# JiahaoPlus/EvoWorld

Measured on AMD Instinct MI355X. Metric: panoramic frames/sec per clip (576x1024x25f, 25 denoise steps), higher is better.
Workload: dtype f16

## Files before the change

### evoworld_amd/_model.py

```python
import json
import math
import os
from collections import OrderedDict
from types import SimpleNamespace

import torch

from . import ops
from .ops import A_CONV3X3, A_CONVT3


class Spec(OrderedDict):

    def add(self, name, shape, kind):
        self[name] = (tuple(shape), kind)

    def conv(self, p, o, i, k):
        self.add(p + ".weight", (o, i) + k, i * math.prod(k))
        self.add(p + ".bias", (o,), i * math.prod(k))

    def lin(self, p, o, i, bias=True):
        self.add(p + ".weight", (o, i), i)
        if bias:
            self.add(p + ".bias", (o,), i)

    def norm(self, p, c):
        self.add(p + ".weight", (c,), "gamma")
        self.add(p + ".bias", (c,), "beta")


class Weights:

    def __init__(self, sd, device):
        self.sd, self.device = sd, device

    def f32(self, k):
        return self.sd[k].to(device=self.device, dtype=torch.float32)

    @staticmethod
    def h(t):
        return t.to(torch.float16).contiguous()

    def pair(self, p):
        return self.h(self.f32(p + ".weight")), self.h(self.f32(p + ".bias"))

    def conv(self, p, cpad=None):
        return ops.pack_conv_weight(self.f32(p + ".weight"), cpad), self.h(self.f32(p + ".bias"))


class PackedModel:
    DEFAULTS = {}
    WEIGHT_FILES = ()
    MISSING = "state dict is missing"
    _spec = _random = None
    PRETRAINED_KW = ()

    def __init__(self, cfg, dtype):
        self._cfg = cfg
        self.config = SimpleNamespace(**cfg)
        self.dtype = dtype
        self.device, self.w = None, None

    @classmethod
    def _config_from_json(cls, raw):
        return {k: raw[k] for k in cls.DEFAULTS if k in raw}

    @classmethod
    def read_config(cls, root):
        cj = os.path.join(root, "config.json")
        if not os.path.exists(cj):
# ... 30 lines not shown
        self.device = torch.device(device)
        if self.device.type != "cuda":
            raise RuntimeError(f"evoworld_amd.{type(self).__name__} needs a GPU device (no CPU path)")
        self._pack(sd)
        return self

    def _require_loaded(self):
        if self.w is None:
            raise RuntimeError("weights not loaded")

    def to(self, *a, **k):
        return self

    def eval(self):
        return self

    def requires_grad_(self, _flag=False):
        return self

    def _conv3x3(self, x, w, b, N, H, W_, Ho, Wo, stride=1, upsample=0, res_out=False, x2=None, c2=None, **kw):
        c1 = x.shape[-1]
        lda2 = x2.shape[-1] if x2 is not None else 0
        M = N * Ho * Wo
        out = self._res(M, w.shape[0], x.device, head="r1" not in kw) if res_out else torch.empty(M, w.shape[0], dtype=torch.float16, device=x.device)
        return ops.gemm(x, w, out, M=M, N=w.shape[0], c1=c1, lda=c1, a2=x2, c2=lda2 if c2 is None else c2, lda2=lda2, bias=b,
                        mode=A_CONV3X3, conv=(N, H, W_, Ho, Wo, stride, upsample), **kw)

    def _convt(self, x, w, b, B, T, P, res_out=False, **kw):
        C = x.shape[-1]
        M = B * T * P
        out = self._res(M, w.shape[0], x.device) if res_out else torch.empty(M, w.shape[0], dtype=torch.float16, device=x.device)
        return ops.gemm(x, w, out, M=M, N=w.shape[0], c1=C, lda=C, bias=b, mode=A_CONVT3, tconv=(B, T, P), **kw)
```

### evoworld_amd/csrc/gemm3_f16.hip

```cpp
#include "gemm_gen23.h"

namespace {

#define EW3_LDS(ptr) (*(const f16x8*)(ptr))

#ifndef EW3_BN
#define EW3_BN 320
#endif
#if EW3_BN == 320
#define EW3_NAME(x) x
#define EW3_KERNEL_STR "gemm3_kernel"
#else
#define EW3_NAME(x) x##_b256
#define EW3_KERNEL_STR "gemm3b_kernel"
#define gemm3_kernel gemm3b_kernel
#endif
constexpr int BM = 256, BN = EW3_BN, BK = 64, NW = 8, WAVES_N = 2;
constexpr int WM = 64, WN = BN / WAVES_N, FM = 4, FN = WN / 16;
static_assert(BN % 64 == 0 && FN % 2 == 0 && (FM * FN) % 8 == 0, "tile geometry");
constexpr int A_BYTES = BM * 128, STAGE = (BM + BN) * 128;
constexpr int GA = BM / 8 / NW, GB = BN / 8 / NW, NP = GA + GB;
constexpr int NSTEP = 2 * FN;
constexpr int ITEMS_BYTES = 8192;
constexpr int PD = 2;
constexpr int BAR_STEP = NSTEP - 1 - PD;


__device__ __forceinline__ void tile_coords(int id, int tiles_m, int tiles_n, int band, int& tm, int& tn) {
    if (band <= 0 || tiles_n <= band) { tm = id / tiles_n; tn = id - tm * tiles_n; return; }
    const int nb = (tiles_n + band - 1) / band;
    const int per_band = band * tiles_m;
    const int k = min(id / per_band, nb - 1);
    const int r = id - k * per_band;
    const int w = k == nb - 1 ? tiles_n - k * band : band;
    tm = r / w;
    tn = k * band + (r - tm * w);
}

template <int MODE, int EPI>
__global__ __launch_bounds__(64 * NW, 2) void gemm3_kernel(const GemmP p, const SkP sk) {
    extern __shared__ __attribute__((aligned(16))) char smem[];
    constexpr bool DIRECT = (EPI & 8) == 0 && (MODE == EW_A_DENSE || (EPI & 16));
#ifndef EW_G3_RESLDS
#define EW_G3_RESLDS 1
#endif
    constexpr bool RB_INIT = DIRECT && (EPI & 1);
    constexpr bool RES_LDS = bool(EW_G3_RESLDS) && DIRECT && (EPI & 6) != 0;
    const int tid = threadIdx.x;
    const int lane = tid & 63;
    const int wave = __builtin_amdgcn_readfirstlane(tid >> 6);
    const int wm = wave / WAVES_N, wn = wave - wm * WAVES_N;
    if (wave >= NW / 2) __builtin_amdgcn_s_setprio(1);

    const int G = gridDim.x;
    const int total_tiles = p.tiles_m * p.tiles_n;
    const int seq0 = (blockIdx.x & 7) * (G >> 3) + (blockIdx.x >> 3);
    const int nk = p.K / BK;
    constexpr bool SK_OK = !(MODE == EW_A_DENSE && EPI == 23);
    const int sk_tiles = SK_OK ? sk.tiles : 0;
// ... 19 lines not shown
            id = (w - n_sk) * G + seq0;
        }
        *(int4*)(items + 4 * w) = make_int4(id, k0, k1, 0);
    }
    __syncthreads();
#define EW3_GET_ITEM(w_, id_, k0_, k1_)                                              \
    do {                                                                             \
        const int4 it__ = *(const int4*)(items + 4 * (w_));                          \
        id_ = __builtin_amdgcn_readfirstlane(it__.x);                                \
        k0_ = __builtin_amdgcn_readfirstlane(it__.y);                                \
        k1_ = __builtin_amdgcn_readfirstlane(it__.z);                                \
    } while (0)

    const int srow = lane >> 3;
    const int slot = (lane & 7) ^ srow;

    constexpr int NTAP = ew_a_ntap<MODE>;
    int ld_w = 0, ld_kt = 0, ld_k1 = 0, ld_tap = 0, ld_cc = 0;
    int a_ctr[GA];
    int a_mask[GA];
    int a_ref = 0;
    unsigned b_off = 0;
    int w_n0 = 0;

    auto loader_new_tile = [&](const int id) __attribute__((always_inline)) {
        int tm, tn;
        tile_coords(id, p.tiles_m, p.tiles_n, p.band, tm, tn);
        const int m0 = tm * BM, n0 = tn * BN;
        int lane_o = lane;
        asm volatile("" : "+v"(lane_o));
        const int srow_o = lane_o >> 3, slot_o = (lane_o & 7) ^ srow_o;
#pragma unroll
        for (int i = 0; i < GA; ++i) {
            int m = m0 + (wave + NW * i) * 8 + srow_o;
            m = m < p.M ? m : p.M - 1;
            int ctr, mask = 1, dcode = 0;
            if constexpr (MODE == EW_A_CONV3X3) {
                const int hw = p.h_out * p.w_out;
                const int img = m / hw, rem = m - img * hw;
                const int oy = rem / p.w_out, ox = rem - oy * p.w_out;
                const int hlim = p.upsample ? 2 * p.h_in : p.h_in, wlim = p.upsample ? 2 * p.w_in : p.w_in;
                const int cy = oy * p.stride + p.conv_shift, cx = ox * p.stride + p.conv_shift;
                mask = 0;
#pragma unroll
                for (int t = 0; t < 9; ++t) {
                    const int iy = cy + t / 3 - 1, ix = cx + t % 3 - 1;
                    if (iy >= 0 && iy < hlim && ix >= 0 && ix < wlim) mask |= 1 << t;
                }
                if (p.upsample) {
                    const int sy = cy >> 1, sx = cx >> 1;
#pragma unroll
                    for (int k = 0; k < 3; ++k) {
                        dcode |= ((((cy + k - 1) >> 1) - sy) + 1) << (2 * k);
                        dcode |= ((((cx + k - 1) >> 1) - sx) + 1) << (6 + 2 * k);
                    }
                    ctr = (img * p.h_in + sy) * p.w_in + sx;
                } else {
                    ctr = (img * p.h_in + cy) * p.w_in + cx;
                }
            } else if constexpr (MODE == EW_A_CONVT3) {
                const int tp = p.tT * p.tP;
                const int bb = m / tp, rem = m - bb * tp;
                const int t = rem / p.tP, x = rem - t * p.tP;
                mask = (t > 0 ? 1 : 0) | 2 | (t + 1 < p.tT ? 4 : 0);
                ctr = (bb * p.tT + t) * p.tP + x;
            } else {
                ctr = m;
            }
            a_mask[i] = mask | (dcode << 16);
            a_ctr[i] = ctr;
        }
        int wrow = wave * 8 + srow_o;
        if constexpr (DIRECT)
            wrow = (wave >> 2) * 32 + ((wave >> 1) & 1) * 4 + (2 * (wave & 1) + (srow_o >> 2)) * 8 + (srow_o & 3);
        b_off = (unsigned)((wrow * p.K + slot_o * 8) * 2);
        w_n0 = n0;
        {
        a_ref = __builtin_amdgcn_readfirstlane(a_ctr[0]);
        if constexpr (MODE == EW_A_CONV3X3) { if (p.upsample) a_ref -= 2 * p.w_in + 1; }
#pragma unroll
        for (int i = 0; i < GA; ++i) a_ctr[i] -= a_ref;
        }
// ... 7 lines not shown
    char* st_buf = smem;
    auto stage_begin = [&](char* buf) __attribute__((always_inline)) {
        bool opened = false;
        if (ld_kt == ld_k1) {
            opened = true;
            int id, k0;
            EW3_GET_ITEM(ld_w, id, k0, ld_k1);
            ++ld_w;
            loader_new_tile(id);
            ld_kt = k0;
            const int chunk = k0 / NTAP;
            ld_tap = k0 - chunk * NTAP;
            ld_cc = chunk * BK;
        }
        st_buf = buf;
        st_tap = ld_tap;
        const int cc = ld_cc;
        const bool second = cc >= p.c1;
        st_base = second ? p.a2 : p.a;
        st_ld = second ? p.lda2 : p.lda;
        st_ch = second ? cc - p.c1 : cc;
        int dpix = ew_a_tap_delta<MODE>(p, st_tap);
        if constexpr (MODE == EW_A_CONV3X3) { if (p.upsample) dpix = 0; }
        const char* ua = (const char*)st_base + ((long long)(a_ref + dpix) * st_ld + st_ch) * 2;
        st_rsrc = __builtin_amdgcn_make_buffer_rsrc((void*)ua, 0, 0x7fffffff, 0x00020000);
        st_ld2 = (unsigned)st_ld * 2u;
        st_wrsrc = __builtin_amdgcn_make_buffer_rsrc((void*)((const char*)p.w + ((size_t)w_n0 * p.K + (size_t)ld_kt * BK) * 2), 0, 0x7fffffff, 0x00020000);
        if (++ld_tap == NTAP) { ld_tap = 0; ld_cc += BK; }
        ++ld_kt;
    };
    auto stage_piece = [&](int k) __attribute__((always_inline)) {
        if (k < GA) {
            const int i = k;
            unsigned rel = (unsigned)a_ctr[i];
            if constexpr (MODE == EW_A_CONV3X3) {
                if (p.upsample) {
                    const int dc = a_mask[i] >> 16;
                    const int dy = ((dc >> (2 * (st_tap / 3))) & 3) - 1, dx = ((dc >> (6 + 2 * (st_tap % 3))) & 3) - 1;
                    rel = (unsigned)(a_ctr[i] + dy * p.w_in + dx);
                }
            }
            unsigned voff = __umul24(rel, st_ld2) + (unsigned)(slot * 16);
            if constexpr (MODE != EW_A_DENSE) voff = ((a_mask[i] >> st_tap) & 1) ? voff : 0x80000000u;
            __builtin_amdgcn_raw_ptr_buffer_load_lds(st_rsrc, (lptr_t)(st_buf + (wave + NW * i) * 1024), 16, (int)voff, 0, 0, 0);
        } else {
            const int j = k - GA;
            __builtin_amdgcn_raw_ptr_buffer_load_lds(st_wrsrc, (lptr_t)(st_buf + A_BYTES + (wave + NW * j) * 1024), 16, (int)b_off, j * (NW * 8 * 2) * p.K, 0, 0);
        }
    };
// ... 4 lines not shown
    for (int kh = 0; kh < 2; ++kh) {
        const int so = ((kh * 4 + fks) ^ sw) << 4;
        a_rd[kh] = (wm * WM + frow) * 128 + so;
        b_rd[kh] = A_BYTES + (wn * WN + frow) * 128 + so;
    }

    f32x4 acc[FM][FN];
    auto init_acc = [&](const int id, const int k0) __attribute__((always_inline)) {
        int tm, tn;
        tile_coords(id, p.tiles_m, p.tiles_n, p.band, tm, tn);
        int lane_o = tid & 63;
        asm volatile("" : "+v"(lane_o));
        const int fks_o = lane_o >> 4;
        const f16* bsrc = (p.bias && k0 == 0) ? p.bias + tn * BN + wn * WN + (DIRECT ? fks_o * 8 : fks_o * 4) : p.zero_page;
        const int on = (p.bias && k0 == 0) ? 1 : 0;
#pragma unroll
        for (int j = 0; j < FN; ++j) {
            const int col = DIRECT ? (j >> 1) * 32 + (j & 1) * 4 : j * 16;
            const f16x4 b4 = *(const f16x4*)(bsrc + col * on);
            const f32x4 b = {(float)b4[0], (float)b4[1], (float)b4[2], (float)b4[3]};
#pragma unroll
            for (int i = 0; i < FM; ++i) acc[i][j] = b;
        }
        if constexpr (RB_INIT) {
            const int frow_o = lane_o & 15;
            const int onr = (p.rowbias && k0 == 0) ? 1 : 0;
#pragma unroll
            for (int i = 0; i < FM; ++i) {
                const int row = min(tm * BM + wm * WM + i * 16 + frow_o, p.M - 1);
                const int g = row / p.rows_per_group;
                const f16* rsrc = onr ? p.rowbias + (size_t)g * p.ld_rowbias + tn * BN + wn * WN + fks_o * 8 : p.zero_page;
#pragma unroll
                for (int j = 0; j < FN; ++j) {
                    const int col = (j >> 1) * 32 + (j & 1) * 4;
                    const f16x4 r4 = *(const f16x4*)(rsrc + col * onr);
                    acc[i][j] += (f32x4){(float)r4[0], (float)r4[1], (float)r4[2], (float)r4[3]};
                }
            }
        }
    };
    f16x8 af[2][FM];
    f16x8 bfr[4];

    stage_begin(stage_base(0));
#pragma unroll
    for (int k = 0; k < NP; ++k) stage_piece(k);
    int staged = 1;
// ... 43 lines not shown
            ew_pin();
#pragma unroll
            for (int i = 0; i < FM; ++i)
                acc[i][j] = __builtin_amdgcn_mfma_f32_16x16x32_f16(bfr[t & 3], af[kh][i], acc[i][j], 0, 0, 0);
            ew_pin();
            if (t == BAR_STEP) {
                ew_wait_vmcnt<0>();
                ew_wait_lgkm0();
                ew_block_barrier();
            }
        }
        s_cur ^= 1;
        if (++cur_kt == cur_k1) {
            const int id = cur_id;
            const bool sk_contribute = SK_OK && cur_tail;
            const bool sk_finish = SK_OK && cur_k1 < nk;
            if (cur_w < n_sk + n_dp) {
                EW3_GET_ITEM(cur_w, cur_id, cur_kt, cur_k1);
                cur_tail = cur_kt > 0;
            }
            ++cur_w;
            int tm, tn;
            tile_coords(id, p.tiles_m, p.tiles_n, p.band, tm, tn);
            const bool full = (tm * BM + wm * WM + WM <= p.M);
            constexpr int CP = WN / 2;
            constexpr int LDP = CP + 4;
            float* patch = (float*)(smem + (s_cur ^ 1) * STAGE) + wave * (16 * LDP);
            const int m_w0 = tm * BM + wm * WM, n_w0 = tn * BN + wn * WN;
            auto epilogue = [&](auto full_tag) __attribute__((always_inline)) {
                constexpr bool FULL = decltype(full_tag)::value;
                int lane = tid & 63;
                asm volatile("" : "+v"(lane));
                const int frow = lane & 15, fks = lane >> 4;
                const f16* bp = p.bias ? p.bias : p.zero_page;
                const f16* rbp = p.rowbias ? p.rowbias : p.zero_page;
                const f16* r1p = p.r1 ? p.r1 : p.zero_page;
                const f16* r2p = p.r2 ? p.r2 : p.zero_page;
                const int mbias = p.bias ? 1 : 0, mrb = p.rowbias ? 1 : 0, m1 = p.r1 ? 1 : 0, m2 = p.r2 ? 1 : 0;
                const int ldrb = p.rowbias ? p.ld_rowbias : 0, ld1 = p.r1 ? p.ld_r1 : 0, ld2 = p.r2 ? p.ld_r2 : 0;
                constexpr int VPR = CP / 8;
                constexpr int ITERS = (16 * VPR + 63) / 64;
                auto is_live = [&](int it) { return it * 64 + lane < 16 * VPR; };
                if constexpr (!DIRECT && (EPI & ~1) == 0) {
                    constexpr bool RB = EPI & 1;
                    constexpr int NH = WN / CP;
                    constexpr int LDH = CP + 8;
// ... 149 lines not shown
                            }
                            if (silu) {
#pragma unroll
                                for (int e = 0; e < 8; ++e) vv[e] = ew_silu(vv[e]);
                            } else if (gelu) {
#pragma unroll
                                for (int e = 0; e < 8; ++e) vv[e] = ew_gelu(vv[e]);
                            }
#pragma unroll
                            for (int e = 0; e < 8; ++e) {
                                float x = vv[e] * p.c_acc;
                                if constexpr (R1 && LO) x += p.c_r1 * ew_split_dec(q1v[st][e], ew_sbyte(q1l[st][e >> 2], e & 3));
                                else if constexpr (R1) x += p.c_r1 * (float)q1v[st][e];
                                if constexpr (R2 && LO) x += p.c_r2 * ew_split_dec(q2v[st][e], ew_sbyte(q2l[st][e >> 2], e & 3));
                                else if constexpr (R2) x += p.c_r2 * (float)q2v[st][e];
                                if constexpr (LO && !R1 && !R2) asm("" : "+v"(x));
                                o[e] = (f16)x;
                                if constexpr (LO) s8[e] = ew_split_enc(x, o[e]);
                            }
                            if constexpr (LO) { ol[0] = ew_pack4(s8[0], s8[1], s8[2], s8[3]); ol[1] = ew_pack4(s8[4], s8[5], s8[6], s8[7]); }
                            ew_pin();
                            if (k + ED < FM * NQ) fetch(k + ED);
                            ew_pin();
                            if ((FULL || m < p.M)) {
                                *(f16x8*)((char*)p.out + (unsigned)(m * p.ld_out + n) * 2u) = o;
                                if constexpr (LO) {
                                    if (p.out_lo) *(u32x2*)((char*)p.out_lo + (unsigned)(m * p.ld_out + n)) = ol;
                                }
                            }
                        }
                    }
                } else {
                    f32x4 bq[FN];
#pragma unroll
                    for (int j = 0; j < FN; ++j) {
                        bq[j] = (f32x4){0.f, 0.f, 0.f, 0.f};
                    }
#pragma unroll
                    for (int i = 0; i < FM; ++i) {
#pragma unroll
                        for (int q = 0; q < FN / 2; ++q) {
                            const f32x4 va = acc[i][2 * q] + bq[2 * q], gg = acc[i][2 * q + 1] + bq[2 * q + 1];
                            const f32x2 o01 = ew_vgelu2((f32x2){va[0], va[1]}, (f32x2){gg[0], gg[1]});
                            const f32x2 o23 = ew_vgelu2((f32x2){va[2], va[3]}, (f32x2){gg[2], gg[3]});
                            const f16x4 o4 = {(f16)o01[0], (f16)o01[1], (f16)o23[0], (f16)o23[1]};
                            *(f16x4*)((f16*)patch + frow * (CP + 8) + q * 16 + fks * 4) = o4;
                        }
                        __builtin_amdgcn_wave_barrier();
#pragma unroll
                        for (int it = 0; it < ITERS; ++it) {
// ... 209 lines not shown
            }
            init_acc(cur_id, cur_kt);
            {
                const char* c2 = stage_base(s_cur);
                {
#pragma unroll
                    for (int i = 0; i < FM; ++i) af[0][i] = EW3_LDS(c2 + a_rd[0] + i * 2048);
                }
#pragma unroll
                for (int j = 0; j < PD; ++j) bfr[j] = EW3_LDS(c2 + b_rd[0] + j * 2048);
            }
        }
    }
}

constexpr int SK_INST = BN == 320 ? 0 : 1;
struct Plan3 {
    int epi, grid;
    GemmP q;
    SkP sk;
    SkWorkspace* w;
};

ew_status plan3(const GemmP& p, hipStream_t s, Plan3& pl, bool* taken) {
    *taken = false;
    if (p.N % BN != 0 || p.M < 320) return EW_OK;
    if (BN != 320 && p.N % 320 == 0) return EW_OK;
    const int NCU = ew_cu_budget();
    const long long tiles = (long long)ew_cdiv(p.M, BM) * (p.N / BN);
    if (tiles > (long long)NCU * (ITEMS_BYTES / 16 - 4)) return EW_OK;
    if (p.act == EW_ACT_GELU && (p.mode != EW_A_DENSE || p.rowbias || p.r1 || p.r2 || p.out_lo)) return EW_OK;
    if (p.act == EW_ACT_SILU && (p.mode != EW_A_DENSE || p.r1 || p.r2 || p.r1_lo || p.r2_lo || p.out_lo)) return EW_OK;
    const long long ld_max = max((long long)p.ld_out, max((long long)p.ld_r1, (long long)p.ld_r2));
    if ((long long)p.M * ld_max * 2 >= (1LL << 32)) return EW_OK;
    if (p.rowbias && ((long long)p.M / max(1, p.rows_per_group) + 2) * p.ld_rowbias * 2 >= (1LL << 32)) return EW_OK;
    if (p.mode == EW_A_DENSE && p.N == BN && p.K <= 1280 && (p.r1 || p.r2)) return EW_OK;
    if (ew_status st = ew_gemm_select_epi(p, 3, &pl.epi)) return st;
    const bool sk_ok = !(p.mode == EW_A_DENSE && pl.epi == 23) && !(p.dbg & 4);
    pl.q = p;
    pl.q.tiles_m = ew_cdiv(p.M, BM); pl.q.tiles_n = p.N / BN;
    pl.q.band = ((long long)p.N * p.K * 2 > 3LL * 1024 * 1024) ? 4 : 0;
    pl.sk = SkP{nullptr, nullptr, 0u, 0, 0}; pl.w = nullptr;
    if (tiles * 256 >= 200LL * NCU) {
        pl.grid = NCU;
        if (tiles < pl.grid) pl.grid = (int)((tiles + 7) / 8 * 8);
        constexpr int sk_min_k = 1280;
        const bool sk_shape = p.mode == EW_A_CONV3X3 || (pl.q.tiles_n <= 2 && p.K >= sk_min_k);
        if (sk_shape && sk_ok && tiles > NCU && tiles % NCU != 0) {
            const long long rounds = (tiles + NCU - 1) / NCU;
            const double loss = 1.0 - (double)tiles / ((double)NCU * rounds);
            if (loss > 0.04 && (pl.w = ew_sk_workspace(SK_INST, s))) {
                pl.sk.dp_rounds = (int)(tiles / NCU) - 1;
                pl.sk.tiles = (int)(tiles - (long long)NCU * pl.sk.dp_rounds);
            }
        }
    } else {
        constexpr int sk_half_min_k = 8192;
        const bool half_shape = tiles >= 8 && 2 * tiles <= NCU && (2 * tiles) % 8 == 0 && (p.K / BK) % 2 == 0 && p.K >= sk_half_min_k;
        if (!sk_ok || p.act == EW_ACT_GEGLU || !half_shape) return EW_OK;
        if (!(pl.w = ew_sk_workspace(SK_INST, s))) return EW_OK;
        pl.grid = (int)(2 * tiles);
        pl.sk.tiles = (int)tiles;
    }
    *taken = true;
    return EW_OK;
}

template <int MODE, int EPI>
ew_status launch3(const Plan3& pl, hipStream_t s) {
    const size_t lds = 2 * STAGE + ITEMS_BYTES;
    static std::atomic<unsigned long long> attr_mask{0};
    if (ew_status st = ew_ensure_dynamic_lds((const void*)gemm3_kernel<MODE, EPI>, (int)lds, attr_mask)) return st;
    SkP sk = pl.sk;
    if (pl.w) ew_sk_begin(SK_INST, pl.w, MODE, EPI, pl.q, &sk);
    ew_gemm_note_kernel(EW3_KERNEL_STR "<%d, %d>", MODE, EPI);
    hipLaunchKernelGGL((gemm3_kernel<MODE, EPI>), dim3(pl.grid), dim3(64 * NW), lds, s, pl.q, sk);
    return ew_check_launch("ew_gemm_f16(gen3)");
}

template <int MODE>
ew_status dispatch_epi3(const Plan3& pl, hipStream_t s) {
    return ew_gemm_visit_variant<3, MODE>(pl.epi, [&](auto e) { return launch3<MODE, decltype(e)::value>(pl, s); });
}

}

const SkInstance EW3_NAME(ew_gemm3_sk) = {EW3_KERNEL_STR, (size_t)FM * FN * 4 * 64 * NW};

ew_status EW3_NAME(ew_gemm3_try)(const GemmP& p, hipStream_t s, bool* taken) {
    Plan3 pl;
    const ew_status st = plan3(p, s, pl, taken);
    if (st || !*taken) return st;
    if (p.mode == EW_A_CONV3X3) return dispatch_epi3<EW_A_CONV3X3>(pl, s);
    if (p.mode == EW_A_CONVT3) return dispatch_epi3<EW_A_CONVT3>(pl, s);
    return dispatch_epi3<EW_A_DENSE>(pl, s);
}
```

### evoworld_amd/csrc/gemm_common.h

```cpp
#pragma once
#include "common.h"

struct GemmP {
    const f16* a;
    const f16* a2;
    const f16* w;
    const f16* bias;
    const f16* rowbias;
    const f16* r1;
    const f16* r2;
    f16* out;
    const f16* zero_page;
    const int8_t* r1_lo;
    const int8_t* r2_lo;
    int8_t* out_lo;
    int M, N, K;
    int c1, c2, lda, lda2, ld_out, ld_r1, ld_r2, ld_rowbias;
    int mode, n_img, h_in, w_in, h_out, w_out, stride, upsample;
    int tB, tT, tP;
    int conv_shift;
    int rows_per_group, act;
    float c_acc, c_r1, c_r2;
    int tiles_m, tiles_n;
    int band;
    int dbg;
};

struct SkP {
    float* ws;
    unsigned* flags;
    unsigned epoch;
    int tiles, dp_rounds;
};

ew_status ew_conv_small_n_try(const GemmP& p, hipStream_t s, bool* taken);
ew_status ew_gemm3_try(const GemmP& p, hipStream_t s, bool* taken);
ew_status ew_gemm3_try_b256(const GemmP& p, hipStream_t s, bool* taken);
ew_status ew_gemm2_dispatch(const GemmP& p, hipStream_t s);
ew_status ew_gemm1_dispatch(const GemmP& p, hipStream_t s);
ew_status ew_gemm_select_epi(const GemmP& p, int generation, int* epi);
void ew_gemm_note_kernel(const char* fmt, ...);
struct SkInstance { const char* kernel; size_t slot_floats; };
extern const SkInstance ew_gemm3_sk, ew_gemm3_sk_b256;
struct SkWorkspace;
SkWorkspace* ew_sk_workspace(int inst, hipStream_t s);
void ew_sk_begin(int inst, SkWorkspace* w, int mode, int epi, const GemmP& p, SkP* sk);

typedef const __attribute__((address_space(1))) void* gptr_t;
typedef __attribute__((address_space(3))) void* lptr_t;

__device__ __forceinline__ void glds16(const f16* src, char* lds_wave_base) {
    __builtin_amdgcn_global_load_lds((gptr_t)src, (lptr_t)lds_wave_base, 16, 0, 0);
}
```

### evoworld_amd/csrc/gemm_dispatch.cpp

```cpp
#include "gemm_common.h"
#include <mutex>

static int g_gemm_gen = -1;
static int g_gemm_dbg = 0;
static char g_gemm_last_kernel[64] = "";
extern "C" const char* ew_gemm_last_kernel(void) { return g_gemm_last_kernel; }
extern "C" void ew_set_gemm_debug(int d) { g_gemm_dbg = d; }
extern "C" void ew_set_gemm_generation(int gen) { g_gemm_gen = gen; }
extern "C" int ew_get_gemm_generation(void) { return g_gemm_gen < 0 ? (g_gemm_gen = 3) : g_gemm_gen; }
void ew_gemm_note_kernel(const char* fmt, ...) {
    va_list ap;
    va_start(ap, fmt);
    vsnprintf(g_gemm_last_kernel, sizeof(g_gemm_last_kernel), fmt, ap);
    va_end(ap);
}

ew_status ew_gemm_select_epi(const GemmP& p, int generation, int* epi) {
    const bool dense = p.mode == EW_A_DENSE;
    if (p.act == EW_ACT_GEGLU && !dense) { ew_set_error("ew_gemm_f16: GEGLU epilogue is only built for dense mode"); return EW_ERR_UNSUPPORTED; }
    if (p.act == EW_ACT_GEGLU) { *epi = 8; return EW_OK; }
    const int mask = (p.rowbias ? 1 : 0) | (p.r1 ? 2 : 0) | (p.r2 ? 4 : 0);
    if (p.r1_lo || p.r2_lo || p.out_lo) {
        if (generation >= 3 && (mask & 6) == 0) *epi = 16 | 1;
        else if (dense) *epi = (mask & 4) == 0 ? 16 | 3 : 16 | 7;
        else if ((mask & 5) == 0) *epi = 16 | 2;
        else if ((mask & 4) == 0) *epi = 16 | 3;
        else { ew_set_error("ew_gemm_f16: conv modes carry the split residual with row-bias / r1 only (no r2)"); return EW_ERR_UNSUPPORTED; }
        return EW_OK;
    }
    if (mask <= 2 || (dense && mask == 3)) *epi = mask;
    else *epi = dense && (mask == 6 || mask == 4) ? 6 : 7;
    return EW_OK;
}

extern "C" ew_status ew_gemm_f16(const ew_gemm_args* a, void* stream) {
    EW_REQUIRE(a != nullptr, "ew_gemm_f16: null args");
    EW_REQUIRE(a->a && a->w && a->out && a->zero_page, "ew_gemm_f16: null a/w/out/zero_page");
    EW_REQUIRE(a->M > 0 && a->N > 0, "ew_gemm_f16: M,N must be > 0 (M=%d N=%d)", a->M, a->N);
    EW_REQUIRE(a->c1 > 0 && a->c1 % 64 == 0 && a->c2 >= 0 && a->c2 % 64 == 0,
               "ew_gemm_f16: c1,c2 must be multiples of 64 (c1=%d c2=%d)", a->c1, a->c2);
    EW_REQUIRE(a->c2 == 0 || a->a2, "ew_gemm_f16: c2 > 0 needs a2");
    EW_REQUIRE(a->N % 4 == 0 && a->ld_out % 4 == 0, "ew_gemm_f16: N and ld_out must be multiples of 4");
    EW_REQUIRE(a->lda % 8 == 0 && (a->c2 == 0 || a->lda2 % 8 == 0), "ew_gemm_f16: lda must be a multiple of 8");
    EW_REQUIRE(a->rows_per_group >= 1, "ew_gemm_f16: rows_per_group must be >= 1");
    EW_REQUIRE(!a->r1 || a->ld_r1 % 4 == 0, "ew_gemm_f16: ld_r1 must be a multiple of 4");
    EW_REQUIRE(!a->r2 || a->ld_r2 % 4 == 0, "ew_gemm_f16: ld_r2 must be a multiple of 4");
    int taps = 1;
    if (a->mode == EW_A_CONV3X3) {
        taps = 9;
        EW_REQUIRE(a->n_img > 0 && a->h_in > 0 && a->w_in > 0 && a->h_out > 0 && a->w_out > 0 &&
                       (a->stride == 1 || a->stride == 2) && (a->upsample == 0 || a->upsample == 1),
                   "ew_gemm_f16: bad conv3x3 geometry");
        EW_REQUIRE((long long)a->n_img * a->h_out * a->w_out == a->M, "ew_gemm_f16: M != n_img*h_out*w_out");
        EW_REQUIRE(!(a->upsample && a->stride != 1), "ew_gemm_f16: upsample needs stride 1");
        EW_REQUIRE((a->conv_shift == 0 || a->conv_shift == 1) && !(a->conv_shift && a->upsample), "ew_gemm_f16: conv_shift must be 0 or 1 (not with upsample)");
    } else if (a->mode == EW_A_CONVT3) {
        taps = 3;
        EW_REQUIRE(a->tB > 0 && a->tT > 0 && a->tP > 0 && (long long)a->tB * a->tT * a->tP == a->M,
                   "ew_gemm_f16: M != B*T*P");
    } else {
        EW_REQUIRE(a->mode == EW_A_DENSE, "ew_gemm_f16: unknown mode %d", a->mode);
    }
    EW_REQUIRE(a->act == EW_ACT_NONE || a->act == EW_ACT_SILU || a->act == EW_ACT_GEGLU || a->act == EW_ACT_GELU, "ew_gemm_f16: unknown act %d", a->act);
    EW_REQUIRE(!a->rowbias || a->ld_rowbias % 4 == 0, "ew_gemm_f16: ld_rowbias must be a multiple of 4");
    if (a->act == EW_ACT_GEGLU)
        EW_REQUIRE(a->N % 128 == 0 && !a->rowbias && !a->r1 && !a->r2 && !a->out_lo, "ew_gemm_f16: GEGLU needs N %% 128 == 0 and no residuals");
    EW_REQUIRE((!a->r1_lo || a->r1) && (!a->r2_lo || a->r2), "ew_gemm_f16: r1_lo / r2_lo need r1 / r2");
    GemmP p;
    p.a = (const f16*)a->a; p.a2 = (const f16*)a->a2; p.w = (const f16*)a->w; p.bias = (const f16*)a->bias;
    p.rowbias = (const f16*)a->rowbias; p.r1 = (const f16*)a->r1; p.r2 = (const f16*)a->r2; p.out = (f16*)a->out;
    p.zero_page = (const f16*)a->zero_page;
    p.r1_lo = (const int8_t*)a->r1_lo; p.r2_lo = (const int8_t*)a->r2_lo; p.out_lo = (int8_t*)a->out_lo;
    p.conv_shift = a->conv_shift;
    p.M = a->M; p.N = a->N; p.K = taps * (a->c1 + a->c2);
    p.c1 = a->c1; p.c2 = a->c2; p.lda = a->lda; p.lda2 = a->lda2; p.ld_out = a->ld_out; p.ld_r1 = a->ld_r1; p.ld_r2 = a->ld_r2; p.ld_rowbias = a->ld_rowbias;
    p.mode = a->mode; p.n_img = a->n_img; p.h_in = a->h_in; p.w_in = a->w_in; p.h_out = a->h_out; p.w_out = a->w_out;
    p.stride = a->stride; p.upsample = a->upsample; p.tB = a->tB; p.tT = a->tT; p.tP = a->tP;
    p.rows_per_group = a->rows_per_group; p.act = a->act; p.c_acc = a->c_acc; p.c_r1 = a->c_r1; p.c_r2 = a->c_r2;
    p.tiles_m = p.tiles_n = 0;
    p.band = 0;
    p.dbg = g_gemm_dbg;
    hipStream_t s = (hipStream_t)stream;
    const int gen = ew_get_gemm_generation();
    bool taken = false;
    ew_status st = EW_OK;
    if (gen >= 2 && ((st = ew_conv_small_n_try(p, s, &taken)) || taken)) return st;
    if (gen >= 3 && ((st = ew_gemm3_try(p, s, &taken)) || taken)) return st;
    if (gen >= 3 && ((st = ew_gemm3_try_b256(p, s, &taken)) || taken)) return st;
    return gen >= 2 ? ew_gemm2_dispatch(p, s) : ew_gemm1_dispatch(p, s);
}

struct SkDesc { unsigned epoch; int mode, epi, M, N, K; };
constexpr int SK_DESC_RING = 1024, SK_SLOTS = 256, SK_POOL = 64;
struct SkWorkspace { int dev; hipStream_t stream; float* ws; unsigned* flags; unsigned epoch; SkDesc* ring; };
struct SkPool {
    const SkInstance& inst;
    SkWorkspace pool[SK_POOL];
    int used = 0;
    std::mutex mutex;
    SkWorkspace* workspace(hipStream_t stream, bool create) {
        std::lock_guard<std::mutex> lock(mutex);
        int dev = 0;
        if (hipGetDevice(&dev) != hipSuccess) return nullptr;
        for (int i = 0; i < used; ++i)
            if (pool[i].dev == dev && pool[i].stream == stream) return &pool[i];
        if (!create || used == SK_POOL) return nullptr;
        SkWorkspace w{dev, stream, nullptr, nullptr, 0, nullptr};
        if (hipExtMallocWithFlags((void**)&w.ws, SK_SLOTS * inst.slot_floats * sizeof(float), hipDeviceMallocUncached) != hipSuccess) { (void)hipGetLastError(); return nullptr; }
// ... 52 lines not shown
```

### evoworld_amd/csrc/gemm_gen23.h

```cpp
#pragma once
#include "gemm_common.h"
#include <type_traits>

template <int MODE>
constexpr int ew_a_ntap = MODE == EW_A_CONV3X3 ? 9 : (MODE == EW_A_CONVT3 ? 3 : 1);

template <int MODE>
__device__ __forceinline__ int ew_a_tap_delta(const GemmP& p, int tap) {
    if constexpr (MODE == EW_A_CONV3X3) return (tap / 3 - 1) * p.w_in + (tap % 3 - 1);
    else if constexpr (MODE == EW_A_CONVT3) return (tap - 1) * p.tP;
    else return 0;
}

template <int GEN, int MODE, class Launch>
ew_status ew_gemm_visit_variant(int epi, Launch&& launch) {
    constexpr bool D = MODE == EW_A_DENSE;
#define EW_VARIANT(E, COMPILED)                                                        \
    case (E):                                                                          \
        if constexpr (COMPILED) return launch(std::integral_constant<int, (E)>{});     \
        break;
    switch (epi) {
        EW_VARIANT(8, D)
        EW_VARIANT(16 | 1, GEN == 3)
        EW_VARIANT(16 | 2, !D)
        EW_VARIANT(16 | 3, true)
        EW_VARIANT(16 | 7, D)
        EW_VARIANT(0, true)
        EW_VARIANT(1, true)
        EW_VARIANT(2, true)
        EW_VARIANT(3, D)
        EW_VARIANT(6, D)
        EW_VARIANT(7, true)
    }
#undef EW_VARIANT
    ew_set_error("ew_gemm_f16: generation %d has no kernel <%d, %d>", GEN, MODE, epi);
    return EW_ERR_UNSUPPORTED;
}
```

### evoworld_amd/ops.py

```python
import ctypes

import numpy as np
import torch

from . import _lib
from ._lib import GemmArgs

A_DENSE, A_CONV3X3, A_CONVT3 = _lib.EW_A_DENSE, _lib.EW_A_CONV3X3, _lib.EW_A_CONVT3
ACT_NONE, ACT_SILU, ACT_GEGLU, ACT_GELU = _lib.EW_ACT_NONE, _lib.EW_ACT_SILU, _lib.EW_ACT_GEGLU, _lib.EW_ACT_GELU

_zero_pages = {}


def _stream():
    return ctypes.c_void_p(torch.cuda.current_stream().cuda_stream)


def _ptr(t):
    return None if t is None else ctypes.c_void_p(t.data_ptr())


def _call(name, *args):
    _lib.check(getattr(_lib.load(), name)(*args, _stream()), name)

# ... 1080 lines not shown
                             f"(got shape {tuple(rowbias.shape)}, strides {tuple(rowbias.stride())})")
        if rowbias.shape[0] < n_groups:
            raise ValueError(f"rowbias has {rowbias.shape[0]} rows; {M} rows in groups of {rows_per_group} need {n_groups}")
    a.x, a.w1p, a.b1p, a.w2p, a.b2, a.rowbias = _ptr(x), _ptr(w1p), _ptr(b1p), _ptr(w2p), _ptr(b2), _ptr(rowbias)
    a.r1, a.r1_lo, a.r2, a.r2_lo, a.out, a.out_lo = _ptr(r1h), _ptr(r1l), _ptr(r2h), _ptr(r2l), _ptr(oh), _ptr(ol)
    a.zero_page = _ptr(zero_page(x.device))
    a.M, a.C, a.hidden = x.shape[0], x.shape[1], w2p.shape[0] * 32
    a.rows_per_group = rows_per_group
    a.ld_rowbias = ld_rowbias
    a.c_acc, a.c_r1, a.c_r2 = c_acc, c_r1, c_r2
    _call("ew_ff_geglu320_f16", ctypes.byref(a))
    return out


def pack_conv_weight(w, cpad=None):
    O, I = w.shape[0], w.shape[1]
    wt = w.reshape(O, I, -1).permute(0, 2, 1)
    if cpad:
        wt = torch.nn.functional.pad(wt, (0, cpad - I))
        I = cpad
    taps = wt.shape[1]
    wt = wt.reshape(O, taps, I // 64, 64).permute(0, 2, 1, 3)
    return wt.reshape(O, -1).to(torch.float16).contiguous()
```

### evoworld_amd/unet.py

```python
import math
import os
from collections import OrderedDict
from types import SimpleNamespace

import torch

from . import ops
from ._model import PackedModel, Spec, Weights
from .ops import ACT_GEGLU, ACT_SILU, Res

DEFAULT_CONFIG = dict(
    sample_size=None, in_channels=18, out_channels=4,
    down_block_types=("CrossAttnDownBlockSpatioTemporal",) * 3 + ("DownBlockSpatioTemporal",),
    up_block_types=("UpBlockSpatioTemporal",) + ("CrossAttnUpBlockSpatioTemporal",) * 3,
    block_out_channels=(320, 640, 1280, 1280), addition_time_embed_dim=256,
    projection_class_embeddings_input_dim=768, layers_per_block=2, cross_attention_dim=1024,
    transformer_layers_per_block=1, num_attention_heads=(5, 10, 20, 20), num_frames=25)

CPAD_IN = 64
SPLIT_DUP_LOG2 = 10


def split_in_offsets(in_channels):
    s = (in_channels + 3) // 4 * 4
# ... 284 lines not shown
            use_fp8 = self._cfg["qkv_fp8"] and c % 64 == 0
            if use_fp8:
                self.fp8_blocks.append(t.p)
            d = {"norm": f.pair(t.p + ".norm"), "proj_in": lin2(t.p + ".proj_in", c, self.split_acts), "proj_out": lin2(t.p + ".proj_out", c),
                 "mix": float(torch.sigmoid(f32(t.p + ".time_mixer.mix_factor")).item()),
                 "pe1": f.pair(t.p + ".time_pos_embed.linear_1"), "pe2": f.pair(t.p + ".time_pos_embed.linear_2")}
            for tag, b in (("s", t.p + ".transformer_blocks.0"), ("t", t.p + ".temporal_transformer_blocks.0")):
                q, k_, v = f32(b + ".attn1.to_q.weight"), f32(b + ".attn1.to_k.weight"), f32(b + ".attn1.to_v.weight")
                if tag == "s":
                    d["s_qk"], d["s_v"] = (fp8(torch.cat([q, k_])), fp8(v)) if use_fp8 else (h(torch.cat([q, k_])), h(v))
                else:
                    d["t_qkv"] = fp8(torch.cat([q, k_, v])) if use_fp8 else h(torch.cat([q, k_, v]))
                    d["t_ff_in"] = ff(b + ".ff_in", b + ".norm_in", c)
                d[tag + "_norm1"], d[tag + "_out"] = f.pair(b + ".norm1"), f.pair(b + ".attn1.to_out.0")
                d[tag + "_ff"] = ff(b + ".ff", b + ".norm3", c)
                cv_w.append(f32(b + ".attn2.to_out.0.weight") @ f32(b + ".attn2.to_v.weight"))
                cv_b.append(f32(b + ".attn2.to_out.0.bias"))
                self._cv_off[(t.p, tag)] = off
                off += c
            W[t.p] = d
        W["cv"] = (h(torch.cat(cv_w)), h(torch.cat(cv_b)))
        self._cv_total = off

        for smp in [blk.down for blk in self.arch.downs if blk.down] + [blk.up for blk in self.arch.ups if blk.up]:
            W[smp.p] = f.conv(smp.p)
        if self.in_split:
            W["conv_in"] = (ops.pack_conv_weight(split_conv_in_weight(f32("conv_in.weight"), self.in_split)), h(f32("conv_in.bias")))
        else:
            W["conv_in"] = f.conv("conv_in", CPAD_IN)
        if self.split_operands:
            w_hi, w_lo = hi_lo(f32("conv_out.weight"))
            W["conv_out"] = (ops.pack_conv_weight(torch.cat([w_hi, w_hi, w_lo] if self.split_acts else [w_hi, w_lo], dim=1)), h(f32("conv_out.bias")))
        else:
            W["conv_out"] = f.conv("conv_out")
        W["norm_out"], W["te1"], W["ae1"] = f.pair("conv_norm_out"), f.pair("time_embedding.linear_1"), f.pair("add_embedding.linear_1")
        W["e2"] = (h(torch.cat([f32("time_embedding.linear_2.weight"), f32("add_embedding.linear_2.weight")], dim=1)),
                   h(f32("time_embedding.linear_2.bias") + f32("add_embedding.linear_2.bias")))
        self.w = W

    def _res(self, rows, C, dev, head=False):
        return Res.empty(rows, C, dev, self.split_heads if head else self.split_residual)

    def _lin2(self, x, w, b, out, **kw):
        C = x.shape[-1]
        if w.shape[1] == C:
            return ops.linear(x, w, b, out=out, **kw)
        c2 = w.shape[1] - C
        return ops.gemm(x, w, out, M=x.shape[0], N=w.shape[0], c1=C, lda=C, a2=x, c2=c2, lda2=C, bias=b, **kw)
# ... 116 lines not shown
                if blk.attn:
                    h = self._transformer(blk.attn[l], h, cvecs, B, T, H, W_)
                skips.append((h, H, W_))
            if blk.down:
                h = self._conv3x3(h.hi, *Wt[blk.down.p], N, H, W_, H // 2, W_ // 2, stride=2, res_out=True)
                H, W_ = H // 2, W_ // 2
                skips.append((h, H, W_))
            if taps is not None:
                taps[f"down{bi}"] = (h.float(), H, W_)
        m = self.arch.mid
        h = self._resblock(m.res[0], [h], tembs, B, T, H, W_)
        h = self._transformer(m.attn[0], h, cvecs, B, T, H, W_)
        h = self._resblock(m.res[1], [h], tembs, B, T, H, W_)
        if taps is not None:
            taps["mid"] = (h.float(), H, W_)
        for bi, blk in enumerate(self.arch.ups):
            for l, r in enumerate(blk.res):
                sk, sh, sw = skips.pop()
                assert (sh, sw) == (H, W_)
                h = self._resblock(r, [h, sk], tembs, B, T, H, W_)
                if blk.attn:
                    h = self._transformer(blk.attn[l], h, cvecs, B, T, H, W_)
            if blk.up:
                h = self._conv3x3(h.hi, *Wt[blk.up.p], N, H, W_, 2 * H, 2 * W_, upsample=1, res_out=True)
                H, W_ = 2 * H, 2 * W_
            if taps is not None:
                taps[f"up{bi}"] = (h.float(), H, W_)
        wco, bco = Wt["conv_out"]
        C0 = h.hi.shape[-1]
        blocks = wco.shape[1] // (9 * C0)
        hn = ops.groupnorm([h], *Wt["norm_out"], N, H * W_, 1e-5, True, pool=self._gn_pool, split_out=blocks == 3)
        return self._conv3x3(hn, wco, bco, N, H, W_, H, W_, x2=hn if blocks > 1 else None, c2=C0 if blocks > 1 else None)

    @torch.no_grad()
    def __call__(self, sample, timestep, encoder_hidden_states, added_time_ids, return_dict=True, taps=None):
        self._require_loaded()
        if sample.ndim != 5 or sample.shape[2] != self._cfg["in_channels"]:
            raise ValueError(f"sample must be [B,T,{self._cfg['in_channels']},h,w], got {tuple(sample.shape)}")
        B, T, C, H, W_ = sample.shape
        if H % 8 or W_ % 8:
            raise ValueError("latent height/width must be multiples of 8 (three stride-2 levels)")
        x = torch.zeros(B * T * H * W_, CPAD_IN, dtype=torch.float16, device=self.device)
        ops.nchw_f32_to_nhwc_f16(sample.to(device=self.device, dtype=torch.float32).reshape(B * T, C, H, W_).contiguous(),
                                 x, CPAD_IN, split=self.in_split)
        eps = self.forward_nhwc(x, timestep, encoder_hidden_states, added_time_ids, B, T, H, W_, taps=taps)
        oc = self._cfg["out_channels"]
        out = ops.nhwc_f16_to_nchw_f32(eps, B * T, oc, H, W_, oc).reshape(B, T, oc, H, W_)
# ... 5 lines not shown
```

### include/evoworld_hip.h

```cpp
#ifndef EVOWORLD_HIP_H
#define EVOWORLD_HIP_H
#include <stddef.h>
#include <stdint.h>
#ifdef __cplusplus
extern "C" {
#endif

typedef int ew_status;
#define EW_OK 0
#define EW_ERR_INVALID_ARG (-1)
#define EW_ERR_UNSUPPORTED (-2)
#define EW_ERR_HIP (-3)

#define EW_ABI_VERSION 20
int ew_abi_version(void);
const char* ew_last_error(void);

enum { EW_A_DENSE = 0, EW_A_CONV3X3 = 1, EW_A_CONVT3 = 2 };
enum { EW_ACT_NONE = 0, EW_ACT_SILU = 1, EW_ACT_GEGLU = 2, EW_ACT_GELU = 3  };

typedef struct ew_gemm_args {
    const void* a;
    const void* a2;
    const void* w;
    const void* bias;
    const void* rowbias;
    const void* r1;
    const void* r2;
    void* out;
    const void* zero_page;
    int M, N;
    int c1, c2;
    int lda, lda2;
    int ld_out, ld_r1, ld_r2, ld_rowbias;
    int mode;
    int n_img, h_in, w_in, h_out, w_out, stride, upsample;
    int tB, tT, tP;
    int rows_per_group;
    int act;
    float c_acc, c_r1, c_r2;
    const void* r1_lo;
    const void* r2_lo;
    void* out_lo;
    int conv_shift;
} ew_gemm_args;

ew_status ew_gemm_f16(const ew_gemm_args* args, void* stream);
void ew_set_gemm_generation(int gen);
int ew_get_gemm_generation(void);
const char* ew_gemm_last_kernel(void);
void ew_set_gemm_debug(int flags);
int ew_gemm_streamk_status(void);
ew_status ew_gemm_streamk_init(void* stream);

int ew_set_cu_budget(int n_cus);
int ew_get_cu_budget(void);
void* ew_stream_create_cu_mask(int first_cu, int n_cus);
ew_status ew_stream_destroy(void* stream);

typedef struct ew_ff_args {
    const void* x;
    const void* w1p;
    const void* b1p;
    const void* w2p;
    const void* b2;
    const void* rowbias;
    const void* r1;
    const void* r1_lo;
    const void* r2;
    const void* r2_lo;
// ... 188 lines not shown
```

Baseline: 5.386.

## Fold nearest-upsample into 3x3 conv as four 2x2 sub-pixel phase convolutions

Replaces the upsample-then-3x3-conv in UNet up blocks with four phase-specific 2x2 convolutions on the low-resolution input. The folded weights are prepacked on the host, and a new CONVUP2 GEMM mode scatters each phase's outputs to the interleaved high-resolution positions. This cuts the reduction depth from 9*C to 4*C per output pixel and skips reading the upsampled image. In exchange it adds a specialized kernel path restricted to N%320 and C%64, and output writes become strided.

```diff
diff --git a/evoworld_amd/_model.py b/evoworld_amd/_model.py
--- a/evoworld_amd/_model.py
+++ b/evoworld_amd/_model.py
@@ -46,6 +46,12 @@
 
     def conv(self, p, cpad=None):
         return ops.pack_conv_weight(self.f32(p + ".weight"), cpad), self.h(self.f32(p + ".bias"))
+
+    def conv_up(self, p):
+        w = self.f32(p + ".weight")
+        if ops.convup2_ok(w.shape[0], w.shape[1]):
+            return ops.pack_convup2_weight(w), self.h(self.f32(p + ".bias")), 2
+        return self.conv(p) + (1,)
 
 
 class PackedModel:
@@ -122,8 +128,9 @@
         c1 = x.shape[-1]
         lda2 = x2.shape[-1] if x2 is not None else 0
         M = N * Ho * Wo
-        out = self._res(M, w.shape[0], x.device, head="r1" not in kw) if res_out else torch.empty(M, w.shape[0], dtype=torch.float16, device=x.device)
-        return ops.gemm(x, w, out, M=M, N=w.shape[0], c1=c1, lda=c1, a2=x2, c2=lda2 if c2 is None else c2, lda2=lda2, bias=b,
+        n_out = w.shape[0] // 4 if upsample == 2 else w.shape[0]
+        out = self._res(M, n_out, x.device, head="r1" not in kw) if res_out else torch.empty(M, n_out, dtype=torch.float16, device=x.device)
+        return ops.gemm(x, w, out, M=M, N=n_out, c1=c1, lda=c1, a2=x2, c2=lda2 if c2 is None else c2, lda2=lda2, bias=b,
                         mode=A_CONV3X3, conv=(N, H, W_, Ho, Wo, stride, upsample), **kw)
 
     def _convt(self, x, w, b, B, T, P, res_out=False, **kw):
diff --git a/evoworld_amd/csrc/gemm3_f16.hip b/evoworld_amd/csrc/gemm3_f16.hip
--- a/evoworld_amd/csrc/gemm3_f16.hip
+++ b/evoworld_amd/csrc/gemm3_f16.hip
@@ -35,6 +35,13 @@
     const int w = k == nb - 1 ? tiles_n - k * band : band;
     tm = r / w;
     tn = k * band + (r - tm * w);
+}
+
+__device__ __forceinline__ int convup2_phase(const GemmP& p, int& tm) {
+    const int per_phase = p.tiles_m >> 2;
+    const int ph = tm / per_phase;
+    tm -= ph * per_phase;
+    return ph;
 }
 
 template <int MODE, int EPI>
@@ -100,10 +107,15 @@
     int a_ref = 0;
     unsigned b_off = 0;
     int w_n0 = 0;
+    int up_ph = 0, up_d0 = 0;
 
     auto loader_new_tile = [&](const int id) __attribute__((always_inline)) {
         int tm, tn;
         tile_coords(id, p.tiles_m, p.tiles_n, p.band, tm, tn);
+        if constexpr (MODE == EW_A_CONVUP2) {
+            up_ph = convup2_phase(p, tm);
+            up_d0 = ((up_ph >> 1) - 1) * p.w_in + (up_ph & 1) - 1;
+        }
         const int m0 = tm * BM, n0 = tn * BN;
         int lane_o = lane;
         asm volatile("" : "+v"(lane_o));
@@ -136,6 +148,17 @@
                 } else {
                     ctr = (img * p.h_in + cy) * p.w_in + cx;
                 }
+            } else if constexpr (MODE == EW_A_CONVUP2) {
+                const int rowi = m / p.w_in;
+                const int sx = m - rowi * p.w_in, sy = rowi % p.h_in;
+                const int y0 = sy + (up_ph >> 1) - 1, x0 = sx + (up_ph & 1) - 1;
+                mask = 0;
+#pragma unroll
+                for (int t = 0; t < 4; ++t) {
+                    const int iy = y0 + (t >> 1), ix = x0 + (t & 1);
+                    if (iy >= 0 && iy < p.h_in && ix >= 0 && ix < p.w_in) mask |= 1 << t;
+                }
+                ctr = m;
             } else if constexpr (MODE == EW_A_CONVT3) {
                 const int tp = p.tT * p.tP;
                 const int bb = m / tp, rem = m - bb * tp;
@@ -189,9 +212,13 @@
         st_ch = second ? cc - p.c1 : cc;
         int dpix = ew_a_tap_delta<MODE>(p, st_tap);
         if constexpr (MODE == EW_A_CONV3X3) { if (p.upsample) dpix = 0; }
+        if constexpr (MODE == EW_A_CONVUP2) dpix += up_d0;
         const char* ua = (const char*)st_base + ((long long)(a_ref + dpix) * st_ld + st_ch) * 2;
         st_rsrc = __builtin_amdgcn_make_buffer_rsrc((void*)ua, 0, 0x7fffffff, 0x00020000);
         st_ld2 = (unsigned)st_ld * 2u;
+        if constexpr (MODE == EW_A_CONVUP2)
+            st_wrsrc = __builtin_amdgcn_make_buffer_rsrc((void*)((const char*)p.w + (((size_t)up_ph * p.N + w_n0) * p.K + (size_t)ld_kt * BK) * 2), 0, 0x7fffffff, 0x00020000);
+        else
         st_wrsrc = __builtin_amdgcn_make_buffer_rsrc((void*)((const char*)p.w + ((size_t)w_n0 * p.K + (size_t)ld_kt * BK) * 2), 0, 0x7fffffff, 0x00020000);
         if (++ld_tap == NTAP) { ld_tap = 0; ld_cc += BK; }
         ++ld_kt;
@@ -242,7 +269,7 @@
 #pragma unroll
             for (int i = 0; i < FM; ++i) acc[i][j] = b;
         }
-        if constexpr (RB_INIT) {
+        if constexpr (RB_INIT && MODE != EW_A_CONVUP2) {
             const int frow_o = lane_o & 15;
             const int onr = (p.rowbias && k0 == 0) ? 1 : 0;
 #pragma unroll
@@ -332,6 +359,8 @@
             ++cur_w;
             int tm, tn;
             tile_coords(id, p.tiles_m, p.tiles_n, p.band, tm, tn);
+            int out_ph = 0;
+            if constexpr (MODE == EW_A_CONVUP2) out_ph = convup2_phase(p, tm);
             const bool full = (tm * BM + wm * WM + WM <= p.M);
             constexpr int CP = WN / 2;
             constexpr int LDP = CP + 4;
@@ -527,10 +556,13 @@
                             ew_pin();
                             if (k + ED < FM * NQ) fetch(k + ED);
                             ew_pin();
+                            int mo = m;
+                            if constexpr (MODE == EW_A_CONVUP2)
+                                mo = 2 * m + 2 * (m / p.w_in) * p.w_in + (out_ph >> 1) * 2 * p.w_in + (out_ph & 1);
                             if ((FULL || m < p.M)) {
-                                *(f16x8*)((char*)p.out + (unsigned)(m * p.ld_out + n) * 2u) = o;
+                                *(f16x8*)((char*)p.out + (unsigned)(mo * p.ld_out + n) * 2u) = o;
                                 if constexpr (LO) {
-                                    if (p.out_lo) *(u32x2*)((char*)p.out_lo + (unsigned)(m * p.ld_out + n)) = ol;
+                                    if (p.out_lo) *(u32x2*)((char*)p.out_lo + (unsigned)(mo * p.ld_out + n)) = ol;
                                 }
                             }
                         }
@@ -786,6 +818,19 @@
     SkWorkspace* w;
 };
 
+void plan3_persistent(Plan3& pl, long long tiles, int NCU, bool tail_ok, hipStream_t s) {
+    pl.grid = NCU;
+    if (tiles < pl.grid) pl.grid = (int)((tiles + 7) / 8 * 8);
+    if (tail_ok && tiles > NCU && tiles % NCU != 0) {
+        const long long rounds = (tiles + NCU - 1) / NCU;
+        const double loss = 1.0 - (double)tiles / ((double)NCU * rounds);
+        if (loss > 0.04 && (pl.w = ew_sk_workspace(SK_INST, s))) {
+            pl.sk.dp_rounds = (int)(tiles / NCU) - 1;
+            pl.sk.tiles = (int)(tiles - (long long)NCU * pl.sk.dp_rounds);
+        }
+    }
+}
+
 ew_status plan3(const GemmP& p, hipStream_t s, Plan3& pl, bool* taken) {
     *taken = false;
     if (p.N % BN != 0 || p.M < 320) return EW_OK;
@@ -806,18 +851,9 @@
     pl.q.band = ((long long)p.N * p.K * 2 > 3LL * 1024 * 1024) ? 4 : 0;
     pl.sk = SkP{nullptr, nullptr, 0u, 0, 0}; pl.w = nullptr;
     if (tiles * 256 >= 200LL * NCU) {
-        pl.grid = NCU;
-        if (tiles < pl.grid) pl.grid = (int)((tiles + 7) / 8 * 8);
         constexpr int sk_min_k = 1280;
         const bool sk_shape = p.mode == EW_A_CONV3X3 || (pl.q.tiles_n <= 2 && p.K >= sk_min_k);
-        if (sk_shape && sk_ok && tiles > NCU && tiles % NCU != 0) {
-            const long long rounds = (tiles + NCU - 1) / NCU;
-            const double loss = 1.0 - (double)tiles / ((double)NCU * rounds);
-            if (loss > 0.04 && (pl.w = ew_sk_workspace(SK_INST, s))) {
-                pl.sk.dp_rounds = (int)(tiles / NCU) - 1;
-                pl.sk.tiles = (int)(tiles - (long long)NCU * pl.sk.dp_rounds);
-            }
-        }
+        plan3_persistent(pl, tiles, NCU, sk_shape && sk_ok, s);
     } else {
         constexpr int sk_half_min_k = 8192;
         const bool half_shape = tiles >= 8 && 2 * tiles <= NCU && (2 * tiles) % 8 == 0 && (p.K / BK) % 2 == 0 && p.K >= sk_half_min_k;
@@ -859,3 +895,23 @@
     if (p.mode == EW_A_CONVT3) return dispatch_epi3<EW_A_CONVT3>(pl, s);
     return dispatch_epi3<EW_A_DENSE>(pl, s);
 }
+
+#if EW3_BN == 320
+ew_status ew_gemm3_convup2(const GemmP& p, hipStream_t s) {
+    Plan3 pl;
+    pl.epi = 16 | 1;
+    pl.q = p;
+    pl.q.M = p.M / 4;
+    pl.q.K = 4 * p.c1;
+    const int NCU = ew_cu_budget();
+    const int per_phase = ew_cdiv(pl.q.M, BM);
+    const long long tiles = 4LL * per_phase * (p.N / BN);
+    EW_REQUIRE(tiles <= (long long)NCU * (ITEMS_BYTES / 16 - 4), "ew_gemm_f16: upsample = 2: %lld tiles exceed the work-item table of %d persistent blocks", tiles, NCU);
+    EW_REQUIRE((long long)p.M * p.ld_out * 2 < (1LL << 32), "ew_gemm_f16: upsample = 2 addresses its output with 32-bit byte offsets (M * ld_out * 2 < 4 GB)");
+    pl.q.tiles_m = 4 * per_phase; pl.q.tiles_n = p.N / BN;
+    pl.q.band = ((long long)p.N * pl.q.K * 2 > 3LL * 1024 * 1024) ? 4 : 0;
+    pl.sk = SkP{nullptr, nullptr, 0u, 0, 0}; pl.w = nullptr;
+    plan3_persistent(pl, tiles, NCU, !(p.dbg & 4), s);
+    return dispatch_epi3<EW_A_CONVUP2>(pl, s);
+}
+#endif
diff --git a/evoworld_amd/csrc/gemm_common.h b/evoworld_amd/csrc/gemm_common.h
--- a/evoworld_amd/csrc/gemm_common.h
+++ b/evoworld_amd/csrc/gemm_common.h
@@ -26,6 +26,8 @@
     int dbg;
 };
 
+constexpr int EW_A_CONVUP2 = 3;
+
 struct SkP {
     float* ws;
     unsigned* flags;
@@ -35,6 +37,7 @@
 
 ew_status ew_conv_small_n_try(const GemmP& p, hipStream_t s, bool* taken);
 ew_status ew_gemm3_try(const GemmP& p, hipStream_t s, bool* taken);
+ew_status ew_gemm3_convup2(const GemmP& p, hipStream_t s);
 ew_status ew_gemm3_try_b256(const GemmP& p, hipStream_t s, bool* taken);
 ew_status ew_gemm2_dispatch(const GemmP& p, hipStream_t s);
 ew_status ew_gemm1_dispatch(const GemmP& p, hipStream_t s);
diff --git a/evoworld_amd/csrc/gemm_dispatch.cpp b/evoworld_amd/csrc/gemm_dispatch.cpp
--- a/evoworld_amd/csrc/gemm_dispatch.cpp
+++ b/evoworld_amd/csrc/gemm_dispatch.cpp
@@ -14,6 +14,8 @@
     vsnprintf(g_gemm_last_kernel, sizeof(g_gemm_last_kernel), fmt, ap);
     va_end(ap);
 }
+
+extern "C" int ew_gemm_convup2_ok(int N, int C) { return N > 0 && N % 320 == 0 && C > 0 && C % 64 == 0; }
 
 ew_status ew_gemm_select_epi(const GemmP& p, int generation, int* epi) {
     const bool dense = p.mode == EW_A_DENSE;
@@ -49,11 +51,18 @@
     if (a->mode == EW_A_CONV3X3) {
         taps = 9;
         EW_REQUIRE(a->n_img > 0 && a->h_in > 0 && a->w_in > 0 && a->h_out > 0 && a->w_out > 0 &&
-                       (a->stride == 1 || a->stride == 2) && (a->upsample == 0 || a->upsample == 1),
+                       (a->stride == 1 || a->stride == 2) && (a->upsample >= 0 && a->upsample <= 2),
                    "ew_gemm_f16: bad conv3x3 geometry");
         EW_REQUIRE((long long)a->n_img * a->h_out * a->w_out == a->M, "ew_gemm_f16: M != n_img*h_out*w_out");
         EW_REQUIRE(!(a->upsample && a->stride != 1), "ew_gemm_f16: upsample needs stride 1");
         EW_REQUIRE((a->conv_shift == 0 || a->conv_shift == 1) && !(a->conv_shift && a->upsample), "ew_gemm_f16: conv_shift must be 0 or 1 (not with upsample)");
+        if (a->upsample == 2) {
+            EW_REQUIRE(!a->a2 && a->c2 == 0, "ew_gemm_f16: upsample = 2 reads one source (no a2 / c2)");
+            EW_REQUIRE(a->h_out == 2 * a->h_in && a->w_out == 2 * a->w_in, "ew_gemm_f16: upsample = 2 needs h_out = 2 h_in and w_out = 2 w_in (got %dx%d -> %dx%d)",
+                       a->h_in, a->w_in, a->h_out, a->w_out);
+            EW_REQUIRE(!a->rowbias && !a->r1 && !a->r2 && a->act == EW_ACT_NONE, "ew_gemm_f16: upsample = 2 is bias + (split) output only: no rowbias / r1 / r2 / act");
+            EW_REQUIRE(ew_gemm_convup2_ok(a->N, a->c1), "ew_gemm_f16: upsample = 2 runs on generation 3's 256x320 tile only: N %% 320 == 0 (N=%d c1=%d)", a->N, a->c1);
+        }
     } else if (a->mode == EW_A_CONVT3) {
         taps = 3;
         EW_REQUIRE(a->tB > 0 && a->tT > 0 && a->tP > 0 && (long long)a->tB * a->tT * a->tP == a->M,
@@ -84,6 +93,7 @@
     const int gen = ew_get_gemm_generation();
     bool taken = false;
     ew_status st = EW_OK;
+    if (p.mode == EW_A_CONV3X3 && p.upsample == 2) return ew_gemm3_convup2(p, s);
     if (gen >= 2 && ((st = ew_conv_small_n_try(p, s, &taken)) || taken)) return st;
     if (gen >= 3 && ((st = ew_gemm3_try(p, s, &taken)) || taken)) return st;
     if (gen >= 3 && ((st = ew_gemm3_try_b256(p, s, &taken)) || taken)) return st;
diff --git a/evoworld_amd/csrc/gemm_gen23.h b/evoworld_amd/csrc/gemm_gen23.h
--- a/evoworld_amd/csrc/gemm_gen23.h
+++ b/evoworld_amd/csrc/gemm_gen23.h
@@ -3,11 +3,12 @@
 #include <type_traits>
 
 template <int MODE>
-constexpr int ew_a_ntap = MODE == EW_A_CONV3X3 ? 9 : (MODE == EW_A_CONVT3 ? 3 : 1);
+constexpr int ew_a_ntap = MODE == EW_A_CONV3X3 ? 9 : (MODE == EW_A_CONVUP2 ? 4 : (MODE == EW_A_CONVT3 ? 3 : 1));
 
 template <int MODE>
 __device__ __forceinline__ int ew_a_tap_delta(const GemmP& p, int tap) {
     if constexpr (MODE == EW_A_CONV3X3) return (tap / 3 - 1) * p.w_in + (tap % 3 - 1);
+    else if constexpr (MODE == EW_A_CONVUP2) return (tap >> 1) * p.w_in + (tap & 1);
     else if constexpr (MODE == EW_A_CONVT3) return (tap - 1) * p.tP;
     else return 0;
 }
@@ -15,6 +16,9 @@
 template <int GEN, int MODE, class Launch>
 ew_status ew_gemm_visit_variant(int epi, Launch&& launch) {
     constexpr bool D = MODE == EW_A_DENSE;
+    if constexpr (MODE == EW_A_CONVUP2) {
+        if (GEN == 3 && epi == (16 | 1)) return launch(std::integral_constant<int, (16 | 1)>{});
+    } else {
 #define EW_VARIANT(E, COMPILED)                                                        \
     case (E):                                                                          \
         if constexpr (COMPILED) return launch(std::integral_constant<int, (E)>{});     \
@@ -32,6 +36,7 @@
         EW_VARIANT(6, D)
         EW_VARIANT(7, true)
     }
+    }
 #undef EW_VARIANT
     ew_set_error("ew_gemm_f16: generation %d has no kernel <%d, %d>", GEN, MODE, epi);
     return EW_ERR_UNSUPPORTED;
diff --git a/evoworld_amd/ops.py b/evoworld_amd/ops.py
--- a/evoworld_amd/ops.py
+++ b/evoworld_amd/ops.py
@@ -1126,3 +1126,26 @@
     taps = wt.shape[1]
     wt = wt.reshape(O, taps, I // 64, 64).permute(0, 2, 1, 3)
     return wt.reshape(O, -1).to(torch.float16).contiguous()
+
+
+CONVUP2_TAPS = (((0,), (1, 2)), ((0, 1), (2,)))
+
+
+def convup2_ok(N, C):
+    return bool(_lib.load().ew_gemm_convup2_ok(int(N), int(C)))
+
+
+def pack_convup2_weight(w, dtype=torch.float16):
+    O, I = w.shape[0], w.shape[1]
+    if tuple(w.shape[2:]) != (3, 3) or I % 64:
+        raise ValueError(f"pack_convup2_weight: expected [O, I % 64 == 0, 3, 3], got {tuple(w.shape)}")
+    ph = w.new_zeros(2, 2, O, 2, 2, I)
+    for a in range(2):
+        for b in range(2):
+            for r in range(2):
+                for c in range(2):
+                    for ky in CONVUP2_TAPS[a][r]:
+                        for kx in CONVUP2_TAPS[b][c]:
+                            ph[a, b, :, r, c] += w[:, :, ky, kx]
+    ph = ph.reshape(4, O, 4, I // 64, 64).permute(0, 1, 3, 2, 4)
+    return ph.reshape(4 * O, 4 * I).to(dtype).contiguous()
diff --git a/evoworld_amd/unet.py b/evoworld_amd/unet.py
--- a/evoworld_amd/unet.py
+++ b/evoworld_amd/unet.py
@@ -330,8 +330,12 @@
         W["cv"] = (h(torch.cat(cv_w)), h(torch.cat(cv_b)))
         self._cv_total = off
 
-        for smp in [blk.down for blk in self.arch.downs if blk.down] + [blk.up for blk in self.arch.ups if blk.up]:
-            W[smp.p] = f.conv(smp.p)
+        for blk in self.arch.downs:
+            if blk.down:
+                W[blk.down.p] = f.conv(blk.down.p)
+        for blk in self.arch.ups:
+            if blk.up:
+                W[blk.up.p] = f.conv_up(blk.up.p)
         if self.in_split:
             W["conv_in"] = (ops.pack_conv_weight(split_conv_in_weight(f32("conv_in.weight"), self.in_split)), h(f32("conv_in.bias")))
         else:
@@ -494,7 +498,8 @@
                 if blk.attn:
                     h = self._transformer(blk.attn[l], h, cvecs, B, T, H, W_)
             if blk.up:
-                h = self._conv3x3(h.hi, *Wt[blk.up.p], N, H, W_, 2 * H, 2 * W_, upsample=1, res_out=True)
+                wu, bu, form = Wt[blk.up.p]
+                h = self._conv3x3(h.hi, wu, bu, N, H, W_, 2 * H, 2 * W_, upsample=form, res_out=True)
                 H, W_ = 2 * H, 2 * W_
             if taps is not None:
                 taps[f"up{bi}"] = (h.float(), H, W_)
diff --git a/include/evoworld_hip.h b/include/evoworld_hip.h
--- a/include/evoworld_hip.h
+++ b/include/evoworld_hip.h
@@ -46,6 +46,7 @@
 } ew_gemm_args;
 
 ew_status ew_gemm_f16(const ew_gemm_args* args, void* stream);
+int ew_gemm_convup2_ok(int N, int C);
 void ew_set_gemm_generation(int gen);
 int ew_get_gemm_generation(void);
 const char* ew_gemm_last_kernel(void);
```

Result: faster. 5.496 (median of 6 runs) (+2.0%).
